# LCSL/nys-koop-lqr

Hardware: AMD Instinct MI355X
Metric: Nyström-Koopman fits/sec (K_nm build + A,B,C solve), N=1e5 m=2000 d=384 (higher is better)
Workload: dtype f64

## Files before the change

### include/nyskoop.h

```cpp
#ifndef NYSKOOP_H
#define NYSKOOP_H

#include <stdint.h>

#ifdef __cplusplus
extern "C" {
#endif

#define NK_ABI_VERSION 2

enum {
  NK_OK = 0,
  NK_ERR_BAD_ARG = -1,
  NK_ERR_HIP = -2,
  NK_ERR_NOT_SPD = -3,
  NK_ERR_OOM = -4,
  NK_ERR_NO_CONVERGENCE = -5,
  NK_ERR_NO_DEVICE = -6
};

enum { NK_KERNEL_RBF = 0, NK_KERNEL_MATERN52 = 1, NK_KERNEL_LINEAR = 2 };

typedef struct nk_kernel_desc {
  int32_t type;
// ... 40 lines not shown
int nk_set_kmat_mode(nk_ctx* ctx, int mode);
int nk_set_strict_spd(nk_ctx* ctx, int strict);
int nk_set_refine(nk_ctx* ctx, double pivot_ratio, int32_t steps);
#define NK_DTYPE_F64 0
#define NK_DTYPE_F32 1
int nk_set_compute_dtype(nk_ctx* ctx, int dtype);
int nk_wait_stream(nk_ctx* ctx, void* producer_stream);
int nk_group_create(int device, int size, nk_ctx** members);
typedef struct nk_cv_unit {
  const nk_kernel_desc* kernel;
  double gamma;
  double jitter;
  int32_t m;
  int32_t reserved;
  int64_t test_begin, test_end;
  const int64_t* landmark_rows;
} nk_cv_unit;
int nk_cv_grid(nk_ctx* const* members, int32_t n_members, const double* X, int64_t ldx, const double* Y, int64_t ldy,
               int64_t n, int32_t d, int32_t p, const nk_cv_unit* units, int32_t n_units, double* scores, int32_t* status);
int nk_group_enter(nk_ctx* member);
int nk_group_leave(nk_ctx* member);
int nk_group_stats(nk_ctx* member, uint64_t* out4);
int nk_runtime_counters(uint64_t* out, int32_t n);
int nk_shutdown(void);

void* nk_host_alloc(uint64_t bytes);
void nk_host_free(void* ptr);

int nk_kernel_matrix(nk_ctx* ctx, const nk_kernel_desc* kd,
                     const double* A, int64_t lda, int64_t nA,
                     const double* B, int64_t ldb, int64_t nB,
                     double* out, int64_t ldo);

int nk_nystrom_fit(nk_ctx* ctx, const nk_kernel_desc* kd,
                   const double* X, int64_t ldx, const double* Y, int64_t ldy,
                   int64_t n, int32_t d, int32_t p,
                   const int64_t* row_ranges, int32_t n_ranges,
                   const double* Zin, int64_t ldzi, const double* Zout, int64_t ldzo, int32_t m,
                   double gamma, double jitter,
                   nk_model** model, nk_fit_stats* stats);

int nk_gram_doubles(int32_t m, int32_t d, int32_t p, int64_t* count);
int nk_nystrom_gram(nk_ctx* ctx, const nk_kernel_desc* kd,
                    const double* X, int64_t ldx, const double* Y, int64_t ldy,
                    int64_t n, int32_t d, int32_t p,
                    const int64_t* row_ranges, int32_t n_ranges,
// ... 56 lines not shown
```

### nys_koop_lqr_amd/_lib.py

```python
import atexit
import ctypes as C
import os
import sys
import threading

import numpy as np

_HERE = os.path.dirname(os.path.abspath(__file__))

NK_KERNEL_RBF, NK_KERNEL_MATERN52, NK_KERNEL_LINEAR = 0, 1, 2
NK_OK = 0
_ERR_NAMES = {-1: "NK_ERR_BAD_ARG", -2: "NK_ERR_HIP", -3: "NK_ERR_NOT_SPD", -4: "NK_ERR_OOM",
              -5: "NK_ERR_NO_CONVERGENCE", -6: "NK_ERR_NO_DEVICE"}


class NyskoopError(RuntimeError):
    def __init__(self, code, msg):
        super().__init__(f"{_ERR_NAMES.get(code, code)}: {msg}")
        self.code = code


class KernelDesc(C.Structure):
    _fields_ = [("type", C.c_int32), ("d", C.c_int32), ("n_lengthscale", C.c_int32), ("reserved", C.c_int32),
                ("lengthscale", C.POINTER(C.c_double)), ("sigma0", C.c_double)]
# ... 22 lines not shown
_I64 = C.c_int64
_I32 = C.c_int32
_D = C.c_double

SIGNATURES = {
    "nk_version": (C.c_int, []),
    "nk_last_error": (C.c_char_p, []),
    "nk_device_count": (C.c_int, []),
    "nk_create": (C.c_int, [C.c_int, C.POINTER(_P)]),
    "nk_destroy": (C.c_int, [_P]),
    "nk_synchronize": (C.c_int, [_P]),
    "nk_stream": (_P, [_P]),
    "nk_set_kmat_mode": (C.c_int, [_P, C.c_int]),
    "nk_set_strict_spd": (C.c_int, [_P, C.c_int]),
    "nk_set_refine": (C.c_int, [_P, C.c_double, C.c_int32]),
    "nk_wait_stream": (C.c_int, [_P, _P]),
    "nk_shutdown": (C.c_int, []),
    "nk_group_create": (C.c_int, [C.c_int, C.c_int, C.POINTER(_P)]),
    "nk_group_enter": (C.c_int, [_P]),
    "nk_group_leave": (C.c_int, [_P]),
    "nk_set_compute_dtype": (C.c_int, [_P, C.c_int]),
    "nk_group_stats": (C.c_int, [_P, C.POINTER(C.c_uint64)]),
    "nk_runtime_counters": (C.c_int, [C.POINTER(C.c_uint64), C.c_int32]),
    "nk_cv_grid": (C.c_int, [C.POINTER(_P), _I32, _P, _I64, _P, _I64, _I64, _I32, _I32, C.POINTER(CvUnit), _I32,
                             C.POINTER(_D), C.POINTER(_I32)]),
    "nk_host_alloc": (_P, [C.c_uint64]),
    "nk_host_free": (None, [_P]),
    "nk_kernel_matrix": (C.c_int, [_P, C.POINTER(KernelDesc), _P, _I64, _I64, _P, _I64, _I64, _P, _I64]),
    "nk_nystrom_fit": (C.c_int, [_P, C.POINTER(KernelDesc), _P, _I64, _P, _I64, _I64, _I32, _I32,
                                 C.POINTER(_I64), _I32, _P, _I64, _P, _I64, _I32, _D, _D,
                                 C.POINTER(_P), C.POINTER(FitStats)]),
    "nk_gram_doubles": (C.c_int, [_I32, _I32, _I32, C.POINTER(_I64)]),
    "nk_nystrom_gram": (C.c_int, [_P, C.POINTER(KernelDesc), _P, _I64, _P, _I64, _I64, _I32, _I32,
                                  C.POINTER(_I64), _I32, _P, _I64, _P, _I64, _I32, _P, C.POINTER(FitStats)]),
    "nk_nystrom_solve": (C.c_int, [_P, C.POINTER(KernelDesc), _P, _I64, _P, _I64, _I32, _I32, _I32, _P, _I64, _D, _D,
                                   C.POINTER(_P), C.POINTER(FitStats)]),
    "nk_model_create": (C.c_int, [_P, C.POINTER(KernelDesc), _P, _I64, _I32, _I32, _I32, _D, _P, _P, _P, _P,
                                  C.POINTER(_P)]),
    "nk_model_destroy": (C.c_int, [_P]),
    "nk_model_get": (C.c_int, [_P, _P, C.c_char, _P, _I64]),
    "nk_model_dims": (C.c_int, [_P, C.POINTER(_I32), C.POINTER(_I32), C.POINTER(_I32)]),
    "nk_model_get_ops": (C.c_int, [_P, _P, _P, _I64, _P, _I64, _P, _I64]),
    "nk_model_get_ops_async": (C.c_int, [_P, _P, _P, _I64, _P, _I64, _P, _I64]),
    "nk_model_wait": (C.c_int, [_P]),
    "nk_lift": (C.c_int, [_P, _P, _P, _I64, _I64, _P, _I64]),
    "nk_predict": (C.c_int, [_P, _P, _P, _I64, _I64, _P, _I64]),
# ... 370 lines not shown
```

### nys_koop_lqr_amd/csrc/nk_api.hip

```cpp
#include "nk_common.h"

#include <cmath>
#include <cstdarg>
#include <cstdio>
#include <cstring>
#include <chrono>
#include <cstdlib>
#include <algorithm>
#include <condition_variable>
#include <mutex>
#include <set>
#include <thread>

namespace nk {

static thread_local std::string g_err;

void set_error(const char* fmt, ...) {
  char buf[1024];
  va_list ap;
  va_start(ap, fmt);
  vsnprintf(buf, sizeof(buf), fmt, ap);
  va_end(ap);
  g_err = buf;
// ... 520 lines not shown
    set_error("nk_group_create: could not create the shared stream / argument table");
    return NK_ERR_HIP;
  }
  for (int i = 0; i < size; ++i) group_attach(g, i, out[i]);
  return NK_OK;
}

int nk_group_enter(nk_ctx* ctx) {
  NK_REQUIRE(ctx != nullptr, "nk_group_enter: null context");
  return group_enter(ctx);
}

int nk_group_leave(nk_ctx* ctx) {
  NK_REQUIRE(ctx != nullptr, "nk_group_leave: null context");
  tl_ctx = ctx;
  const int rc = group_leave(ctx);
  tl_ctx = nullptr;
  return rc;
}

int nk_runtime_counters(uint64_t* out, int32_t n) {
  NK_REQUIRE(out != nullptr && n >= 0, "nk_runtime_counters: bad argument");
  for (int i = 0; i < n && i < CNT_N; ++i) out[i] = nk::read_counter(i);
  return NK_OK;
}

int nk_group_stats(nk_ctx* ctx, uint64_t* out4) {
  NK_REQUIRE(ctx != nullptr && out4 != nullptr, "nk_group_stats: null argument");
  group_stats(ctx, out4);
  return NK_OK;
}

int nk_cv_grid(nk_ctx* const* members, int32_t n_members, const double* X, int64_t ldx, const double* Y, int64_t ldy,
               int64_t n, int32_t d, int32_t p, const nk_cv_unit* units, int32_t n_units, double* scores, int32_t* status) {
  NK_REQUIRE(members && n_members >= 1 && X && Y && units && scores, "nk_cv_grid: null argument");
  NK_REQUIRE(n > 0 && d > 0 && p >= 0 && n_units >= 0 && ldx >= d + p && ldy >= d, "nk_cv_grid: bad sizes");
  for (int k = 0; k < n_members; ++k) NK_REQUIRE(members[k] != nullptr, "nk_cv_grid: null member context");
  for (int u = 0; u < n_units; ++u) {
    const nk_cv_unit& cu = units[u];
    NK_REQUIRE(cu.kernel && cu.landmark_rows && cu.m > 0, "nk_cv_grid: unit %d: null kernel / landmarks", u);
    NK_REQUIRE(0 <= cu.test_begin && cu.test_begin < cu.test_end && cu.test_end <= n, "nk_cv_grid: unit %d: bad test fold", u);
    for (int j = 0; j < cu.m; ++j)
      NK_REQUIRE(cu.landmark_rows[j] >= 0 && cu.landmark_rows[j] < n, "nk_cv_grid: unit %d: landmark row out of range", u);
  }
  if (n_units == 0) return NK_OK;
  nk_ctx* lead = members[0];
// ... 1562 lines not shown
```

### nys_koop_lqr_amd/csrc/nk_chol_flow.hip

```cpp
#include "nk_common.h"
#include "nk_panel_body.h"
#include "nk_potrf_body.h"

namespace nk {

namespace {

constexpr int FLOW_THREADS = 256;
constexpr int FLOW_HDR = 16;
constexpr int FLOW_POLL_LIMIT = 1 << 22;

struct FlowSys {
  double* P;
  int64_t ldp;
  int m, extra;
  double* Linv;
  double* pivlog;
  int* info;
  unsigned long long* piv;
  int* flags;
  int nblk;
  int nex;
};
struct FlowArgs {
  FlowSys s[2];
  int nsys;
  int total;
  int fix;
  int* hdr;
};

__device__ __forceinline__ int ld_flag(const int* f) { return __hip_atomic_load(f, __ATOMIC_RELAXED, __HIP_MEMORY_SCOPE_AGENT); }

__device__ __forceinline__ int col_items(const FlowSys& s, int c) {
  if (c < 0 || c >= s.nblk) return 0;
  return max(0, s.nblk - c - 2) + s.nex;
}

__device__ void item_of(const FlowArgs& a, int t, int& q, int& i, int& k) {
  for (int g = 0;; ++g) {
    for (int p = 0; p < a.nsys; ++p)
      if (g < a.s[p].nblk) {
        if (t == 0) { q = p; i = k = g; return; }
        --t;
      }
    for (int p = 0; p < a.nsys; ++p) {
      const int n = col_items(a.s[p], g - 1);
      if (t < n) {
        q = p; k = g - 1;
        const int nsq = max(0, a.s[p].nblk - k - 2);
        i = t < nsq ? k + 2 + t : a.s[p].nblk + (t - nsq);
// ... 123 lines not shown
    __hip_atomic_store(s.flags + i * s.nblk + k, 1, __ATOMIC_RELAXED, __HIP_MEMORY_SCOPE_AGENT);
  }
}

__device__ __forceinline__ void local_sync() {
  asm volatile("s_waitcnt vmcnt(0)" ::: "memory");
  __syncthreads();
}

__device__ __forceinline__ void panel_tile(const FlowArgs& a, const FlowSys& s, int r0, int r1, int k, int wave, int lane) {
  PanelSys ps;
  ps.P = s.P + (int64_t)r0 * s.ldp + CHOL_NB * k;
  ps.ldp = s.ldp;
  ps.Linv = s.Linv + (size_t)k * CHOL_WS;
  ps.rows = r1 - r0;
  ps.nb = min(CHOL_NB, s.m - CHOL_NB * k);
  ps.fix = a.fix;
  ps.nblocks = 1;
  chol_panel_rows(ps, 16 * wave, lane);
  __builtin_amdgcn_s_setprio(0);
}

__device__ __noinline__ void flow_potrf(double* A, int64_t lda, int nb, double* Linv, int* info, unsigned long long* piv,
                                       double* plog, int blk, int lane) {
  PotrfBatch pb;
  pb.A[0] = A; pb.lda[0] = lda; pb.nb[0] = nb; pb.Linv[0] = Linv; pb.info[0] = info; pb.piv[0] = piv; pb.plog[0] = plog;
  pb.A[1] = nullptr; pb.lda[1] = 0; pb.nb[1] = 0; pb.Linv[1] = nullptr; pb.info[1] = nullptr; pb.piv[1] = nullptr;
  pb.plog[1] = nullptr;
  potrf_diag_kernel_body<true>(pb, blk, 0, lane);
  __builtin_amdgcn_s_setprio(0);
}

__global__ void __launch_bounds__(FLOW_THREADS) chol_flow_kernel(FlowArgs a) {
  __shared__ int sh[4];
  const int lane = threadIdx.x & 63;
  const int wave = __builtin_amdgcn_readfirstlane(threadIdx.x >> 6);
  const int wm = wave >> 1, wn = wave & 1;
  const int l15 = lane & 15, l4 = lane >> 4;
  for (;;) {
    if (threadIdx.x == 0) sh[1] = atomicAdd(a.hdr, 1);
    __syncthreads();
    const int t = sh[1];
    __syncthreads();
    if (t >= a.total) return;
    int q = 0, i = 0, k = 0;
    item_of(a, t, q, i, k);
    const FlowSys s = q ? a.s[1] : a.s[0];
    int r0, r1;
    tile_rows(s, i, r0, r1);
    const int c0 = CHOL_NB * k, c1 = min(c0 + CHOL_NB, s.m);
    if (i == k) {
      if (k > 0) {
        const int p0 = c0 - CHOL_NB;
        Quarter Cp, Cd;
        load_quarter(s, r0, r1, p0, c0, wm, wn, l15, l4, Cp);
        load_quarter(s, r0, r1, c0, c1, wm, wn, l15, l4, Cd);
        bool ok = true;
        for (int j = 0; j < k - 1 && ok;) {
          const int J = wait_tiles(a, s, k, k - 1, j, k - 1, sh);
          if (J < 0) { ok = false; break; }
          for (; j < J; ++j) {
            update_quarter(s, r0, r1, p0, c0, j, wm, wn, l15, l4, Cp);
            update_quarter(s, r0, r1, c0, c1, j, wm, wn, l15, l4, Cd);
          }
        }
        if (!ok) continue;
        store_quarter(s, r0, r1, p0, c0, wm, wn, l15, l4, Cp);
        store_quarter(s, r0, r1, c0, c1, wm, wn, l15, l4, Cd);
        local_sync();
        if (wait_tiles(a, s, k - 1, -1, k - 1, k, sh) < 0) continue;
        panel_tile(a, s, r0, r1, k - 1, wave, lane);
        publish(s, k, k - 1);
        __syncthreads();
        load_quarter(s, r0, r1, c0, c1, wm, wn, l15, l4, Cd);
        update_quarter(s, r0, r1, c0, c1, k - 1, wm, wn, l15, l4, Cd);
        store_quarter(s, r0, r1, c0, c1, wm, wn, l15, l4, Cd);
        local_sync();
      }
      if (wave == 0)
        flow_potrf(s.P + (int64_t)c0 * s.ldp + c0, s.ldp, c1 - c0, s.Linv + (size_t)k * CHOL_WS, s.info, s.piv,
                   s.pivlog ? s.pivlog + c0 : nullptr, k, lane);
      publish(s, k, k);
      __syncthreads();
    } else {
      if (k > 0) {
        Quarter C;
        load_quarter(s, r0, r1, c0, c1, wm, wn, l15, l4, C);
        bool ok = true;
        for (int j = 0; j < k && ok;) {
          const int J = wait_tiles(a, s, i, k, j, k, sh);
          if (J < 0) { ok = false; break; }
          for (; j < J; ++j) update_quarter(s, r0, r1, c0, c1, j, wm, wn, l15, l4, C);
        }
        if (!ok) continue;
        store_quarter(s, r0, r1, c0, c1, wm, wn, l15, l4, C);
        local_sync();
      }
      if (wait_tiles(a, s, k, -1, k, k + 1, sh) < 0) continue;
      panel_tile(a, s, r0, r1, k, wave, lane);
      publish(s, i, k);
      __syncthreads();
    }
  }
}

}

bool chol_flow_enabled() {
  const char* e = getenv("NYSKOOP_CHOL_FLOW");
  return !(e && e[0] == '0');
}

int cholesky_flow_pair(nk_ctx* ctx, const CholSys* sys, int nsys) {
  constexpr int NB = CHOL_NB;
  NK_REQUIRE(nsys >= 1 && nsys <= 2, "cholesky_flow_pair: 1..2 systems");
  FlowArgs a;
  memset(&a, 0, sizeof(a));
  a.nsys = nsys;
  a.fix = chol_fix_enabled();
  size_t words = FLOW_HDR;
  for (int q = 0; q < nsys; ++q) {
    const CholSys& y = sys[q];
    FlowSys& s = a.s[q];
    s.P = y.P; s.ldp = y.ldp; s.m = y.m; s.extra = y.extra; s.Linv = y.Linv; s.pivlog = y.pivlog;
    s.info = ctx->d_info + info_base(ctx) + q;
    s.piv = ctx->d_piv + 2 * (info_base(ctx) + q);
    s.nblk = (y.m + NB - 1) / NB;
    s.nex = (y.extra + NB - 1) / NB;
    words += (size_t)(s.nblk + s.nex) * s.nblk;
    for (int c = 0; c < s.nblk; ++c) a.total += 1 + std::max(0, s.nblk - c - 2) + s.nex;
  }
  const int slot = info_base(ctx) / 2;
  if (ctx->flow_words[slot] < words) {
    if (ctx->d_flow[slot]) NK_HIP(hipFree(ctx->d_flow[slot]));
    ctx->d_flow[slot] = nullptr;
    ctx->flow_words[slot] = 0;
    NK_HIP(hipMalloc(reinterpret_cast<void**>(&ctx->d_flow[slot]), words * sizeof(int)));
    ctx->flow_words[slot] = words;
  }
  a.hdr = ctx->d_flow[slot];
  int* f = a.hdr + FLOW_HDR;
  for (int q = 0; q < nsys; ++q) {
    a.s[q].flags = f;
    f += (size_t)(a.s[q].nblk + a.s[q].nex) * a.s[q].nblk;
  }
  NK_HIP(hipMemsetAsync(a.hdr, 0, words * sizeof(int), ctx->stream));
  const int grid = std::max(1, std::min(a.total, ctx->num_cu / 2));
  hipLaunchKernelGGL(chol_flow_kernel, dim3((unsigned)grid), dim3(FLOW_THREADS), 0, ctx->stream, a);
  NK_HIP(hipGetLastError());
  count_event(CNT_CHOL_FLOW);
  return NK_OK;
}

}
```

### nys_koop_lqr_amd/csrc/nk_common.h

```cpp
#pragma once
#include <hip/hip_runtime.h>
#include <stdint.h>
#include <stddef.h>
#include <string>
#include <vector>

#include "nyskoop.h"
#include "nk_lockstep.h"

namespace nk {

void set_error(const char* fmt, ...);

#define NK_HIP(call)                                                                         \
  do {                                                                                       \
    hipError_t e_ = (call);                                                                  \
    if (e_ != hipSuccess) {                                                                  \
      nk::set_error("%s failed: %s (%s:%d)", #call, hipGetErrorString(e_), __FILE__, __LINE__); \
      return e_ == hipErrorOutOfMemory ? NK_ERR_OOM : NK_ERR_HIP;                            \
    }                                                                                        \
  } while (0)

#define NK_TRY(call)            \
  do {                          \
// ... 39 lines not shown
  hipStream_t stream_la[2] = {nullptr, nullptr};
  hipEvent_t ev_la[2][4] = {};
  int compute_f32 = 0;
  hipEvent_t ev_fork = nullptr, ev_join = nullptr, ev_chain = nullptr;
  int* d_info = nullptr;
  unsigned long long* d_piv = nullptr;
  unsigned long long* h_piv = nullptr;
  double* d_scalars = nullptr;
  double* h_scalars = nullptr;
  int* h_info = nullptr;
  double* d_zeros = nullptr;
  hipEvent_t ev[16];
  int num_cu = 256;
  int kmat_mode = 0;
  double refine_pivot = 0.0;
  int refine_steps = 2;
  int strict_spd = 0;
  hipEvent_t ev_ext = nullptr;
  hipEvent_t ev_up[8] = {};
  nk_group* group = nullptr;
  nk_member_state* gstate = nullptr;
  int* d_flow[2] = {nullptr, nullptr};
  size_t flow_words[2] = {0, 0};
  bool chol_flow_off = false;
  double* h_stage = nullptr;
  size_t h_stage_bytes = 0;
};

struct nk_model {
  int device = 0;
  int32_t m = 0, d = 0, p = 0;
  int32_t ktype = 0;
  double sigma0 = 0.0;
  double jitter = 0.0;
  double* buf = nullptr;
  size_t bytes = 0;
  double *A = nullptr, *B = nullptr, *C = nullptr, *W = nullptr, *S = nullptr, *Sinv = nullptr, *Z = nullptr,
         *winv = nullptr;
  bool has_ops = false;
  hipEvent_t ev_fetch = nullptr;
};

namespace nk {

struct SideScope {
  nk_ctx* c;
// ... 131 lines not shown
int sqrtm_finish(nk_ctx* ctx, SqrtPlan* plan, double* S, double* Sinv);
int sqrtm_verdict(nk_ctx* ctx, SqrtPlan* plan, int* iters, double* resid);
int cholesky_lower(nk_ctx* ctx, double* P, int64_t ldp, int m, double* Linv );
int cholesky_solve(nk_ctx* ctx, const double* L, int64_t ldl, int m, const double* Linv, double* R, int64_t ldr,
                   int nrhs);
struct CholSys {
  double* P = nullptr;
  int64_t ldp = 0;
  int m = 0;
  int extra = 0;
  bool backward = true;
  double* Linv = nullptr;
  double* pivlog = nullptr;
  double* R = nullptr;
  int64_t ldr = 0;
  int nrhs = 0;
};
int cholesky_lower_pair(nk_ctx* ctx, const CholSys* sys, int nsys);
int cholesky_lower_pair_async(nk_ctx* ctx, const CholSys* sys, int nsys);
int cholesky_check_pair(nk_ctx* ctx, const CholSys* sys, int nsys);
int cholesky_solve_pair(nk_ctx* ctx, const CholSys* sys, int nsys);
int cholesky_aug_pair_async(nk_ctx* ctx, const CholSys* sys, int nsys, hipEvent_t pause = nullptr, int pause_step = -1);
constexpr int CHOL_NB = 64;
constexpr int CHOL_WS = 2 * CHOL_NB * CHOL_NB + 8;
constexpr double CHOL_FIX_KAPPA = 8.0 * CHOL_NB;
inline int chol_fix_enabled() {
  const char* e = getenv("NYSKOOP_CHOL_FIX");
  return (e && e[0] == '0') ? 0 : ((e && e[0] == '2') ? 2 : 1);
}
bool launch_chol_trail_pair(nk_ctx* ctx, const GemmCall* calls, int ncalls, int* rc);
bool launch_chol_trail_potrf_pair(nk_ctx* ctx, const GemmCall* calls, int ncalls, const int* nb, double* const* Linv, int blk,
                                  double* const* plog, int* rc);
inline bool chol_fuse_enabled() {
  const char* e = getenv("NYSKOOP_CHOL_FUSE");
  return !(e && e[0] == '0');
}
bool chol_flow_enabled();
int cholesky_flow_pair(nk_ctx* ctx, const CholSys* sys, int nsys);
constexpr int CHOL_FLOW_GIVEUP = -0x40000000;
bool launch_chol_panel_pair(nk_ctx* ctx, const GemmCall* calls, int ncalls, int* rc);
int launch_trsm_right_lower_pair(nk_ctx* ctx, const CholSys* sys, int nsys);

struct PinvInfo {
  int rank = 0, sweeps = 0;
  bool converged = false;
  double sigma_max = 0.0, sigma_min_kept = 0.0, sigma_min = 0.0;
// ... 130 lines not shown
```

### nys_koop_lqr_amd/csrc/nk_potrf_body.h

```cpp
#pragma once
#include "nk_common.h"

namespace nk {

typedef double d4 __attribute__((ext_vector_type(4)));

__device__ __forceinline__ double readlane_f64(double v, int lane) {
  const int lo = __builtin_amdgcn_readlane(__double2loint(v), lane);
  const int hi = __builtin_amdgcn_readlane(__double2hiint(v), lane);
  return __hiloint2double(hi, lo);
}

struct PotrfBatch {
  double* A[2];
  int64_t lda[2];
  int nb[2];
  double* Linv[2];
  int* info[2];
  unsigned long long* piv[2];
  double* plog[2];
};

constexpr int PLD = CHOL_NB + 1;
constexpr int SLD = 17;
// ... 5 lines not shown
    double a = P[l15 * ldp + 4 * ks + l4];
    const double b = Q[(4 * ks + l4) * ldq + l15];
    if (NEG) a = -a;
    acc = __builtin_amdgcn_mfma_f64_16x16x4f64(a, b, acc, 0, 0, 0);
  }
  return acc;
}
__device__ __forceinline__ void store_tile(double* T, int ldt, d4 acc, int l15, int l4) {
#pragma unroll
  for (int reg = 0; reg < 4; ++reg) T[(l4 + 4 * reg) * ldt + l15] = acc[reg];
}

template <bool WAVE_SYNC>
__device__ __forceinline__ void potrf_sync() {
  if (WAVE_SYNC) {
    __builtin_amdgcn_fence(__ATOMIC_RELEASE, "workgroup");
    __builtin_amdgcn_wave_barrier();
    __builtin_amdgcn_fence(__ATOMIC_ACQUIRE, "workgroup");
  } else {
    __syncthreads();
  }
}

template <bool WAVE_SYNC = false>
__device__ __forceinline__ void potrf_diag_kernel_body(const PotrfBatch& pb, int blk, int which, int lane) {
  constexpr int NB = CHOL_NB;
  static_assert(NB == 64, "one lane per row, four 16-column panels");
  const int nb = pb.nb[which];
  if (nb <= 0) return;
  __builtin_amdgcn_s_setprio(3);
  double* __restrict__ A = pb.A[which];
  const int64_t lda = pb.lda[which];
  double* __restrict__ Linv = pb.Linv[which];
  int* __restrict__ info = pb.info[which];
  double* __restrict__ plog = pb.plog[which];
  double piv_min = 1.0e308, piv_max = 0.0;
  __shared__ double As[NB * PLD];
  __shared__ double Iv[NB * PLD];
  __shared__ double Sc[3 * 16 * SLD];
  __shared__ double dinv[NB];
  const int l15 = lane & 15, l4 = lane >> 4;
#pragma unroll 8
  for (int r = 0; r < NB; ++r) {
    double v = (r == lane) ? 1.0 : 0.0;
    if (r < nb && lane < nb) v = A[(int64_t)r * lda + lane];
    As[r * PLD + lane] = v;
  }
  potrf_sync<WAVE_SYNC>();

#pragma unroll
  for (int pbk = 0; pbk < 4; ++pbk) {
    const int c0 = 16 * pbk;
    double R[16];
#pragma unroll
    for (int jj = 0; jj < 16; ++jj) R[jj] = As[lane * PLD + c0 + jj];
#pragma unroll
    for (int k = 0; k < 16; ++k) {
      double dkk = readlane_f64(R[k], c0 + k);
      if (lane == 0 && plog != nullptr && c0 + k < nb) plog[c0 + k] = dkk;
      if (!(dkk > 0.0) || !isfinite(dkk)) {
        if (lane == 0 && c0 + k < nb) atomicCAS(info, 0, blk * NB + c0 + k + 1);
        dkk = 1.0;
      } else if (c0 + k < nb) {
        piv_min = fmin(piv_min, dkk);
        piv_max = fmax(piv_max, dkk);
      }
      double inv = __builtin_amdgcn_rsq(dkk);
      inv = inv * fma(-0.5 * dkk * inv, inv, 1.5);
      inv = inv * fma(-0.5 * dkk * inv, inv, 1.5);
      double s = dkk * inv;
      s = fma(0.5 * inv, fma(-s, s, dkk), s);
      inv = fma(inv, fma(-s, inv, 1.0), inv);
      if (lane == c0 + k) dinv[c0 + k] = inv;
      R[k] = (lane == c0 + k) ? s : R[k] * inv;
      {
        const int rk_lo = __double2loint(R[k]), rk_hi = __double2hiint(R[k]);
#pragma unroll
        for (int jj = k + 1; jj < 16; ++jj)
          asm volatile("v_readlane_b32 s96, %1, %3\n\tv_readlane_b32 s97, %2, %3\n\ts_nop 0\n\tv_fma_f64 %0, -%4, s[96:97], %0"
                       : "+v"(R[jj])
                       : "v"(rk_lo), "v"(rk_hi), "i"(c0 + jj), "v"(R[k])
                       : "s96", "s97");
      }
    }
#pragma unroll
    for (int jj = 0; jj < 16; ++jj) As[lane * PLD + c0 + jj] = R[jj];
    potrf_sync<WAVE_SYNC>();
#pragma unroll
    for (int ti = pbk + 1; ti < 4; ++ti)
#pragma unroll
      for (int tj = pbk + 1; tj <= ti; ++tj) {
        d4 c;
#pragma unroll
        for (int reg = 0; reg < 4; ++reg) c[reg] = As[(16 * ti + l4 + 4 * reg) * PLD + 16 * tj + l15];
#pragma unroll
        for (int ks = 0; ks < 4; ++ks) {
          const double a = -As[(16 * ti + l15) * PLD + c0 + 4 * ks + l4];
          const double b = As[(16 * tj + l15) * PLD + c0 + 4 * ks + l4];
          c = __builtin_amdgcn_mfma_f64_16x16x4f64(a, b, c, 0, 0, 0);
        }
#pragma unroll
        for (int reg = 0; reg < 4; ++reg) As[(16 * ti + l4 + 4 * reg) * PLD + 16 * tj + l15] = c[reg];
      }
    potrf_sync<WAVE_SYNC>();
  }
#pragma unroll 8
  for (int r = 0; r < NB; ++r)
    if (r < nb && lane < nb) A[(int64_t)r * lda + lane] = As[r * PLD + lane];

  {
    const double* Lb = As + (16 * l4) * PLD + 16 * l4;
    double x[16];
#pragma unroll
    for (int i = 0; i < 16; ++i) {
      double s0 = (i == l15) ? 1.0 : 0.0, s1 = 0.0;
#pragma unroll
      for (int j = 0; j < i; ++j) {
        const double l = Lb[i * PLD + j];
        if ((j & 1) == 0) s0 = fma(-l, x[j], s0);
        else s1 = fma(-l, x[j], s1);
      }
      x[i] = (s0 + s1) * dinv[16 * l4 + i];
    }
    double* Db = Iv + (16 * l4) * PLD + 16 * l4;
#pragma unroll
    for (int i = 0; i < 16; ++i) Db[i * PLD + l15] = x[i];
  }
  potrf_sync<WAVE_SYNC>();
  auto Lblk = [&](int i, int j) { return As + (16 * i) * PLD + 16 * j; };
  auto Xblk = [&](int i, int j) { return Iv + (16 * i) * PLD + 16 * j; };
  const d4 zero = d4{0.0, 0.0, 0.0, 0.0};
#pragma unroll
  for (int i = 1; i < 4; ++i)
    store_tile(Sc + (i - 1) * 16 * SLD, SLD, mm16<false>(Lblk(i, i - 1), PLD, Xblk(i - 1, i - 1), PLD, zero, l15, l4), l15, l4);
  potrf_sync<WAVE_SYNC>();
#pragma unroll
  for (int i = 1; i < 4; ++i)
    store_tile(Xblk(i, i - 1), PLD, mm16<true>(Xblk(i, i), PLD, Sc + (i - 1) * 16 * SLD, SLD, zero, l15, l4), l15, l4);
  potrf_sync<WAVE_SYNC>();
#pragma unroll
  for (int i = 2; i < 4; ++i) {
    d4 t = mm16<false>(Lblk(i, i - 2), PLD, Xblk(i - 2, i - 2), PLD, zero, l15, l4);
    t = mm16<false>(Lblk(i, i - 1), PLD, Xblk(i - 1, i - 2), PLD, t, l15, l4);
    store_tile(Sc + (i - 2) * 16 * SLD, SLD, t, l15, l4);
  }
  potrf_sync<WAVE_SYNC>();
#pragma unroll
  for (int i = 2; i < 4; ++i)
    store_tile(Xblk(i, i - 2), PLD, mm16<true>(Xblk(i, i), PLD, Sc + (i - 2) * 16 * SLD, SLD, zero, l15, l4), l15, l4);
  potrf_sync<WAVE_SYNC>();
  {
    d4 t = mm16<false>(Lblk(3, 0), PLD, Xblk(0, 0), PLD, zero, l15, l4);
    t = mm16<false>(Lblk(3, 1), PLD, Xblk(1, 0), PLD, t, l15, l4);
    t = mm16<false>(Lblk(3, 2), PLD, Xblk(2, 0), PLD, t, l15, l4);
    store_tile(Sc, SLD, t, l15, l4);
  }
  potrf_sync<WAVE_SYNC>();
  store_tile(Xblk(3, 0), PLD, mm16<true>(Xblk(3, 3), PLD, Sc, SLD, zero, l15, l4), l15, l4);
  potrf_sync<WAVE_SYNC>();
#pragma unroll 8
  for (int i = 0; i < NB; ++i) Linv[i * NB + lane] = (l4 <= (i >> 4)) ? Iv[i * PLD + lane] : 0.0;
  double sl = 0.0, si = 0.0;
#pragma unroll 8
  for (int i = 0; i < NB; ++i) {
    const double vl = (lane <= i) ? As[i * PLD + lane] : 0.0;
    const double vi = (l4 <= (i >> 4)) ? Iv[i * PLD + lane] : 0.0;
    Linv[NB * NB + i * NB + lane] = vl;
    sl = fma(vl, vl, sl);
    si = fma(vi, vi, si);
  }
#pragma unroll
  for (int off = 32; off > 0; off >>= 1) {
    sl += __shfl_xor(sl, off, 64);
    si += __shfl_xor(si, off, 64);
  }
  if (lane == 0) Linv[2 * NB * NB] = (sl * si > CHOL_FIX_KAPPA * CHOL_FIX_KAPPA) ? 1.0 : 0.0;
  if (lane == 0 && piv_max > 0.0) {
    atomicMin(pb.piv[which], (unsigned long long)__double_as_longlong(piv_min));
    atomicMax(pb.piv[which] + 1, (unsigned long long)__double_as_longlong(piv_max));
  }
}
}
```

Baseline: 24.49.

## Factor flow diagonal block with all four waves, keeping updated tile in LDS

By default the Cholesky flow kernel now factors each diagonal 64x64 block with all four waves instead of wave 0 alone. The panel factorisation on wave 0 runs alongside the blocked triangular inverse on wave 1, and the trailing MFMA tile updates are spread across waves. The updated diagonal quarter now stays in LDS rather than making a round-trip through global memory, and is written back only after publish. Optional wall-clock stamps and an nk_flow_stamps API are added for profiling, and the old single-wave path is kept behind NYSKOOP_FLOW_DIAG=1. The catch is extra __syncthreads inside the block and a more complex dependency order in the inverse computation.

```diff
diff --git a/include/nyskoop.h b/include/nyskoop.h
--- a/include/nyskoop.h
+++ b/include/nyskoop.h
@@ -86,6 +86,7 @@
 int nk_group_leave(nk_ctx* member);
 int nk_group_stats(nk_ctx* member, uint64_t* out4);
 int nk_runtime_counters(uint64_t* out, int32_t n);
+int nk_flow_stamps(nk_ctx* ctx, int32_t slot, uint64_t* out, int32_t n, int32_t* meta);
 int nk_shutdown(void);
 
 void* nk_host_alloc(uint64_t bytes);
diff --git a/nys_koop_lqr_amd/_lib.py b/nys_koop_lqr_amd/_lib.py
--- a/nys_koop_lqr_amd/_lib.py
+++ b/nys_koop_lqr_amd/_lib.py
@@ -68,6 +68,7 @@
     "nk_set_compute_dtype": (C.c_int, [_P, C.c_int]),
     "nk_group_stats": (C.c_int, [_P, C.POINTER(C.c_uint64)]),
     "nk_runtime_counters": (C.c_int, [C.POINTER(C.c_uint64), C.c_int32]),
+    "nk_flow_stamps": (C.c_int, [_P, _I32, C.POINTER(C.c_uint64), _I32, C.POINTER(_I32)]),
     "nk_cv_grid": (C.c_int, [C.POINTER(_P), _I32, _P, _I64, _P, _I64, _I64, _I32, _I32, C.POINTER(CvUnit), _I32,
                              C.POINTER(_D), C.POINTER(_I32)]),
     "nk_host_alloc": (_P, [C.c_uint64]),
diff --git a/nys_koop_lqr_amd/csrc/nk_api.hip b/nys_koop_lqr_amd/csrc/nk_api.hip
--- a/nys_koop_lqr_amd/csrc/nk_api.hip
+++ b/nys_koop_lqr_amd/csrc/nk_api.hip
@@ -566,6 +566,29 @@
 int nk_runtime_counters(uint64_t* out, int32_t n) {
   NK_REQUIRE(out != nullptr && n >= 0, "nk_runtime_counters: bad argument");
   for (int i = 0; i < n && i < CNT_N; ++i) out[i] = nk::read_counter(i);
+  return NK_OK;
+}
+
+int nk_flow_stamps(nk_ctx* ctx, int32_t slot, uint64_t* out, int32_t n, int32_t* meta) {
+  NK_TRY(check_ctx(ctx));
+  NK_REQUIRE(slot >= 0 && slot < 2 && out != nullptr && n >= 0 && meta != nullptr, "nk_flow_stamps: bad argument");
+  NK_HIP(hipSetDevice(ctx->device));
+  for (hipStream_t q : {ctx->stream_main, ctx->stream_side, ctx->stream_prep})
+    if (q) NK_HIP(hipStreamSynchronize(q));
+  const bool on = ctx->flow_stamp_off[slot] != 0;
+  meta[0] = on ? ctx->flow_stamp_nblk[slot][0] : 0;
+  meta[1] = on ? ctx->flow_stamp_nblk[slot][1] : 0;
+  meta[2] = FLOW_NST;
+  int khz = 0;
+  NK_HIP(hipDeviceGetAttribute(&khz, hipDeviceAttributeWallClockRate, ctx->device));
+  meta[3] = khz;
+  const size_t total = (size_t)(meta[0] + meta[1]) * FLOW_NST;
+  if (on && total > 0 && n > 0)
+  {
+    NK_HIP(hipMemcpyAsync(out, ctx->d_flow[slot] + ctx->flow_stamp_off[slot], std::min(total, (size_t)n) * sizeof(uint64_t),
+                          hipMemcpyDeviceToHost, ctx->stream_main));
+    NK_HIP(hipStreamSynchronize(ctx->stream_main));
+  }
   return NK_OK;
 }
 
diff --git a/nys_koop_lqr_amd/csrc/nk_chol_flow.hip b/nys_koop_lqr_amd/csrc/nk_chol_flow.hip
--- a/nys_koop_lqr_amd/csrc/nk_chol_flow.hip
+++ b/nys_koop_lqr_amd/csrc/nk_chol_flow.hip
@@ -21,12 +21,14 @@
   int* flags;
   int nblk;
   int nex;
+  unsigned long long* stamps;
 };
 struct FlowArgs {
   FlowSys s[2];
   int nsys;
   int total;
   int fix;
+  int diag1;
   int* hdr;
 };
 
@@ -196,13 +198,65 @@
 }
 
 __device__ __noinline__ void flow_potrf(double* A, int64_t lda, int nb, double* Linv, int* info, unsigned long long* piv,
-                                       double* plog, int blk, int lane) {
+                                       double* plog, int blk, int lane, unsigned long long* st) {
   PotrfBatch pb;
   pb.A[0] = A; pb.lda[0] = lda; pb.nb[0] = nb; pb.Linv[0] = Linv; pb.info[0] = info; pb.piv[0] = piv; pb.plog[0] = plog;
   pb.A[1] = nullptr; pb.lda[1] = 0; pb.nb[1] = 0; pb.Linv[1] = nullptr; pb.info[1] = nullptr; pb.piv[1] = nullptr;
   pb.plog[1] = nullptr;
-  potrf_diag_kernel_body<true>(pb, blk, 0, lane);
+  potrf_diag_kernel_body<true>(pb, blk, 0, lane, st);
   __builtin_amdgcn_s_setprio(0);
+}
+
+__device__ __forceinline__ void flow_diag_load(const double* A, int64_t lda, int nb, int wave, int lane) {
+  double* As = potrf_lds().As;
+#pragma unroll
+  for (int rr = 0; rr < 16; ++rr) {
+    const int r = 16 * wave + rr;
+    double v = (r == lane) ? 1.0 : 0.0;
+    if (r < nb && lane < nb) v = A[(int64_t)r * lda + lane];
+    As[r * PLD + lane] = v;
+  }
+}
+__device__ __noinline__ void flow_diag4(const double* A, int64_t lda, int nb, double* Linv, int* info, unsigned long long* piv,
+                                        double* plog, int blk, int wave, int lane, unsigned long long* st) {
+  if (A != nullptr) flow_diag_load(A, lda, nb, wave, lane);
+  __syncthreads();
+  potrf_stamp(st, 4);
+  potrf_diag_flow_body(nb, Linv, info, piv, plog, blk, wave, lane, st);
+  __builtin_amdgcn_s_setprio(0);
+}
+
+template <bool PAD>
+__device__ __forceinline__ void quarter_to_lds(const Quarter& C, int nb, int wm, int wn, int l15, int l4) {
+  double* As = potrf_lds().As;
+#pragma unroll
+  for (int a = 0; a < 2; ++a)
+#pragma unroll
+    for (int b = 0; b < 2; ++b)
+#pragma unroll
+      for (int reg = 0; reg < 4; ++reg) {
+        const int row = 32 * wm + 16 * a + l4 + 4 * reg, col = 32 * wn + 16 * b + l15;
+        double v = C[a][b][reg];
+        if (PAD && !(row < nb && col < nb)) v = (row == col) ? 1.0 : 0.0;
+        As[row * PLD + col] = v;
+      }
+}
+__device__ __forceinline__ void quarter_from_lds(Quarter& C, int wm, int wn, int l15, int l4) {
+  const double* As = potrf_lds().As;
+#pragma unroll
+  for (int a = 0; a < 2; ++a)
+#pragma unroll
+    for (int b = 0; b < 2; ++b)
+#pragma unroll
+      for (int reg = 0; reg < 4; ++reg) C[a][b][reg] = As[(32 * wm + 16 * a + l4 + 4 * reg) * PLD + 32 * wn + 16 * b + l15];
+}
+__device__ __forceinline__ void flow_diag_writeback(double* A, int64_t lda, int nb, int wave, int lane) {
+  const double* As = potrf_lds().As;
+#pragma unroll
+  for (int rr = 0; rr < 16; ++rr) {
+    const int r = 16 * wave + rr;
+    if (r < nb && lane < nb) A[(int64_t)r * lda + lane] = As[r * PLD + lane];
+  }
 }
 
 __global__ void __launch_bounds__(FLOW_THREADS) chol_flow_kernel(FlowArgs a) {
@@ -224,6 +278,10 @@
     tile_rows(s, i, r0, r1);
     const int c0 = CHOL_NB * k, c1 = min(c0 + CHOL_NB, s.m);
     if (i == k) {
+      unsigned long long* st = s.stamps ? s.stamps + (size_t)k * FLOW_NST : nullptr;
+      potrf_stamp(st, 0);
+      const int nb = c1 - c0;
+      double* Akk = s.P + (int64_t)c0 * s.ldp + c0;
       if (k > 0) {
         const int p0 = c0 - CHOL_NB;
         Quarter Cp, Cd;
@@ -239,23 +297,42 @@
           }
         }
         if (!ok) continue;
+        potrf_stamp(st, 1);
         store_quarter(s, r0, r1, p0, c0, wm, wn, l15, l4, Cp);
-        store_quarter(s, r0, r1, c0, c1, wm, wn, l15, l4, Cd);
+        if (a.diag1) store_quarter(s, r0, r1, c0, c1, wm, wn, l15, l4, Cd);
+        else quarter_to_lds<false>(Cd, nb, wm, wn, l15, l4);
         local_sync();
         if (wait_tiles(a, s, k - 1, -1, k - 1, k, sh) < 0) continue;
+        potrf_stamp(st, 2);
         panel_tile(a, s, r0, r1, k - 1, wave, lane);
         publish(s, k, k - 1);
         __syncthreads();
-        load_quarter(s, r0, r1, c0, c1, wm, wn, l15, l4, Cd);
-        update_quarter(s, r0, r1, c0, c1, k - 1, wm, wn, l15, l4, Cd);
-        store_quarter(s, r0, r1, c0, c1, wm, wn, l15, l4, Cd);
-        local_sync();
-      }
-      if (wave == 0)
-        flow_potrf(s.P + (int64_t)c0 * s.ldp + c0, s.ldp, c1 - c0, s.Linv + (size_t)k * CHOL_WS, s.info, s.piv,
-                   s.pivlog ? s.pivlog + c0 : nullptr, k, lane);
+        potrf_stamp(st, 3);
+        if (a.diag1) {
+          load_quarter(s, r0, r1, c0, c1, wm, wn, l15, l4, Cd);
+          update_quarter(s, r0, r1, c0, c1, k - 1, wm, wn, l15, l4, Cd);
+          store_quarter(s, r0, r1, c0, c1, wm, wn, l15, l4, Cd);
+          local_sync();
+        } else {
+          quarter_from_lds(Cd, wm, wn, l15, l4);
+          update_quarter(s, r0, r1, c0, c1, k - 1, wm, wn, l15, l4, Cd);
+          quarter_to_lds<true>(Cd, nb, wm, wn, l15, l4);
+        }
+      }
+      double* plog = s.pivlog ? s.pivlog + c0 : nullptr;
+      double* Lk = s.Linv + (size_t)k * CHOL_WS;
+      if (a.diag1) {
+        if (wave == 0) flow_potrf(Akk, s.ldp, nb, Lk, s.info, s.piv, plog, k, lane, st);
+      } else {
+        flow_diag4(k == 0 ? Akk : nullptr, s.ldp, nb, Lk, s.info, s.piv, plog, k, wave, lane, st);
+      }
       publish(s, k, k);
       __syncthreads();
+      potrf_stamp(st, 10);
+      if (!a.diag1) {
+        flow_diag_writeback(Akk, s.ldp, nb, wave, lane);
+        potrf_stamp(st, 11);
+      }
     } else {
       if (k > 0) {
         Quarter C;
@@ -280,6 +357,11 @@
 
 }
 
+static bool env_is_1(const char* name) {
+  const char* e = getenv(name);
+  return e && e[0] == '1';
+}
+
 bool chol_flow_enabled() {
   const char* e = getenv("NYSKOOP_CHOL_FLOW");
   return !(e && e[0] == '0');
@@ -292,6 +374,8 @@
   memset(&a, 0, sizeof(a));
   a.nsys = nsys;
   a.fix = chol_fix_enabled();
+  a.diag1 = env_is_1("NYSKOOP_FLOW_DIAG");
+  const bool stamps = env_is_1("NYSKOOP_FLOW_STAMPS");
   size_t words = FLOW_HDR;
   for (int q = 0; q < nsys; ++q) {
     const CholSys& y = sys[q];
@@ -302,6 +386,7 @@
     s.nblk = (y.m + NB - 1) / NB;
     s.nex = (y.extra + NB - 1) / NB;
     words += (size_t)(s.nblk + s.nex) * s.nblk;
+    if (stamps) words += 2 * (size_t)s.nblk * FLOW_NST + 1;
     for (int c = 0; c < s.nblk; ++c) a.total += 1 + std::max(0, s.nblk - c - 2) + s.nex;
   }
   const int slot = info_base(ctx) / 2;
@@ -318,6 +403,18 @@
     a.s[q].flags = f;
     f += (size_t)(a.s[q].nblk + a.s[q].nex) * a.s[q].nblk;
   }
+  ctx->flow_stamp_off[slot] = 0;
+  if (stamps) {
+    ctx->flow_stamp_off[slot] = (f - a.hdr + 1) & ~(size_t)1;
+    unsigned long long* st = reinterpret_cast<unsigned long long*>(a.hdr + ctx->flow_stamp_off[slot]);
+    for (int q = 0; q < 2; ++q) {
+      ctx->flow_stamp_nblk[slot][q] = q < nsys ? a.s[q].nblk : 0;
+      if (q < nsys) {
+        a.s[q].stamps = st;
+        st += (size_t)a.s[q].nblk * FLOW_NST;
+      }
+    }
+  }
   NK_HIP(hipMemsetAsync(a.hdr, 0, words * sizeof(int), ctx->stream));
   const int grid = std::max(1, std::min(a.total, ctx->num_cu / 2));
   hipLaunchKernelGGL(chol_flow_kernel, dim3((unsigned)grid), dim3(FLOW_THREADS), 0, ctx->stream, a);
diff --git a/nys_koop_lqr_amd/csrc/nk_common.h b/nys_koop_lqr_amd/csrc/nk_common.h
--- a/nys_koop_lqr_amd/csrc/nk_common.h
+++ b/nys_koop_lqr_amd/csrc/nk_common.h
@@ -85,6 +85,8 @@
   nk_member_state* gstate = nullptr;
   int* d_flow[2] = {nullptr, nullptr};
   size_t flow_words[2] = {0, 0};
+  size_t flow_stamp_off[2] = {0, 0};
+  int flow_stamp_nblk[2][2] = {{0, 0}, {0, 0}};
   bool chol_flow_off = false;
   double* h_stage = nullptr;
   size_t h_stage_bytes = 0;
@@ -262,6 +264,7 @@
 int cholesky_solve_pair(nk_ctx* ctx, const CholSys* sys, int nsys);
 int cholesky_aug_pair_async(nk_ctx* ctx, const CholSys* sys, int nsys, hipEvent_t pause = nullptr, int pause_step = -1);
 constexpr int CHOL_NB = 64;
+constexpr int FLOW_NST = 16;
 constexpr int CHOL_WS = 2 * CHOL_NB * CHOL_NB + 8;
 constexpr double CHOL_FIX_KAPPA = 8.0 * CHOL_NB;
 inline int chol_fix_enabled() {
diff --git a/nys_koop_lqr_amd/csrc/nk_potrf_body.h b/nys_koop_lqr_amd/csrc/nk_potrf_body.h
--- a/nys_koop_lqr_amd/csrc/nk_potrf_body.h
+++ b/nys_koop_lqr_amd/csrc/nk_potrf_body.h
@@ -51,8 +51,100 @@
   }
 }
 
+struct PotrfLds {
+  double As[CHOL_NB * PLD];
+  double Iv[CHOL_NB * PLD];
+  double Sc[3 * 16 * SLD];
+  double dinv[CHOL_NB];
+};
+__device__ __forceinline__ PotrfLds& potrf_lds() {
+  __shared__ PotrfLds s;
+  return s;
+}
+
+__device__ __forceinline__ void potrf_stamp(unsigned long long* st, int slot) {
+  if (st != nullptr && threadIdx.x == 0) st[slot] = (unsigned long long)wall_clock64();
+}
+
+__device__ __forceinline__ void potrf_panel(double* As, double* dinv, int pbk, int lane, int nb, int blk, int* info, double* plog,
+                                            double& piv_min, double& piv_max) {
+  constexpr int NB = CHOL_NB;
+  const int c0 = 16 * pbk;
+  double R[16];
+#pragma unroll
+  for (int jj = 0; jj < 16; ++jj) R[jj] = As[lane * PLD + c0 + jj];
+#pragma unroll
+  for (int k = 0; k < 16; ++k) {
+    double dkk = readlane_f64(R[k], c0 + k);
+    if (lane == 0 && plog != nullptr && c0 + k < nb) plog[c0 + k] = dkk;
+    if (!(dkk > 0.0) || !isfinite(dkk)) {
+      if (lane == 0 && c0 + k < nb) atomicCAS(info, 0, blk * NB + c0 + k + 1);
+      dkk = 1.0;
+    } else if (c0 + k < nb) {
+      piv_min = fmin(piv_min, dkk);
+      piv_max = fmax(piv_max, dkk);
+    }
+    double inv = __builtin_amdgcn_rsq(dkk);
+    inv = inv * fma(-0.5 * dkk * inv, inv, 1.5);
+    inv = inv * fma(-0.5 * dkk * inv, inv, 1.5);
+    double s = dkk * inv;
+    s = fma(0.5 * inv, fma(-s, s, dkk), s);
+    inv = fma(inv, fma(-s, inv, 1.0), inv);
+    if (lane == c0 + k) dinv[c0 + k] = inv;
+    R[k] = (lane == c0 + k) ? s : R[k] * inv;
+    {
+      const int rk_lo = __double2loint(R[k]), rk_hi = __double2hiint(R[k]);
+#pragma unroll
+      for (int jj = k + 1; jj < 16; ++jj)
+        asm volatile("v_readlane_b32 s96, %1, %3\n\tv_readlane_b32 s97, %2, %3\n\ts_nop 0\n\tv_fma_f64 %0, -%4, s[96:97], %0"
+                     : "+v"(R[jj])
+                     : "v"(rk_lo), "v"(rk_hi), "i"(c0 + jj), "v"(R[k])
+                     : "s96", "s97");
+    }
+  }
+#pragma unroll
+  for (int jj = 0; jj < 16; ++jj) As[lane * PLD + c0 + jj] = R[jj];
+}
+
+__device__ __forceinline__ void potrf_tile_update(double* As, int pbk, int ti, int tj, int l15, int l4) {
+  const int c0 = 16 * pbk;
+  d4 c;
+#pragma unroll
+  for (int reg = 0; reg < 4; ++reg) c[reg] = As[(16 * ti + l4 + 4 * reg) * PLD + 16 * tj + l15];
+#pragma unroll
+  for (int ks = 0; ks < 4; ++ks) {
+    const double a = -As[(16 * ti + l15) * PLD + c0 + 4 * ks + l4];
+    const double b = As[(16 * tj + l15) * PLD + c0 + 4 * ks + l4];
+    c = __builtin_amdgcn_mfma_f64_16x16x4f64(a, b, c, 0, 0, 0);
+  }
+#pragma unroll
+  for (int reg = 0; reg < 4; ++reg) As[(16 * ti + l4 + 4 * reg) * PLD + 16 * tj + l15] = c[reg];
+}
+
+__device__ __forceinline__ void potrf_inv_diag(const double* As, double* Iv, const double* dinv, int b, int l15, bool store) {
+  const double* Lb = As + (16 * b) * PLD + 16 * b;
+  double x[16];
+#pragma unroll
+  for (int i = 0; i < 16; ++i) {
+    double s0 = (i == l15) ? 1.0 : 0.0, s1 = 0.0;
+#pragma unroll
+    for (int j = 0; j < i; ++j) {
+      const double l = Lb[i * PLD + j];
+      if ((j & 1) == 0) s0 = fma(-l, x[j], s0);
+      else s1 = fma(-l, x[j], s1);
+    }
+    x[i] = (s0 + s1) * dinv[16 * b + i];
+  }
+  if (store) {
+    double* Db = Iv + (16 * b) * PLD + 16 * b;
+#pragma unroll
+    for (int i = 0; i < 16; ++i) Db[i * PLD + l15] = x[i];
+  }
+}
+
 template <bool WAVE_SYNC = false>
-__device__ __forceinline__ void potrf_diag_kernel_body(const PotrfBatch& pb, int blk, int which, int lane) {
+__device__ __forceinline__ void potrf_diag_kernel_body(const PotrfBatch& pb, int blk, int which, int lane,
+                                                       unsigned long long* st = nullptr) {
   constexpr int NB = CHOL_NB;
   static_assert(NB == 64, "one lane per row, four 16-column panels");
   const int nb = pb.nb[which];
@@ -64,10 +156,11 @@
   int* __restrict__ info = pb.info[which];
   double* __restrict__ plog = pb.plog[which];
   double piv_min = 1.0e308, piv_max = 0.0;
-  __shared__ double As[NB * PLD];
-  __shared__ double Iv[NB * PLD];
-  __shared__ double Sc[3 * 16 * SLD];
-  __shared__ double dinv[NB];
+  PotrfLds& lds = potrf_lds();
+  double* As = lds.As;
+  double* Iv = lds.Iv;
+  double* Sc = lds.Sc;
+  double* dinv = lds.dinv;
   const int l15 = lane & 15, l4 = lane >> 4;
 #pragma unroll 8
   for (int r = 0; r < NB; ++r) {
@@ -76,85 +169,24 @@
     As[r * PLD + lane] = v;
   }
   potrf_sync<WAVE_SYNC>();
+  potrf_stamp(st, 4);
 
 #pragma unroll
   for (int pbk = 0; pbk < 4; ++pbk) {
-    const int c0 = 16 * pbk;
-    double R[16];
-#pragma unroll
-    for (int jj = 0; jj < 16; ++jj) R[jj] = As[lane * PLD + c0 + jj];
-#pragma unroll
-    for (int k = 0; k < 16; ++k) {
-      double dkk = readlane_f64(R[k], c0 + k);
-      if (lane == 0 && plog != nullptr && c0 + k < nb) plog[c0 + k] = dkk;
-      if (!(dkk > 0.0) || !isfinite(dkk)) {
-        if (lane == 0 && c0 + k < nb) atomicCAS(info, 0, blk * NB + c0 + k + 1);
-        dkk = 1.0;
-      } else if (c0 + k < nb) {
-        piv_min = fmin(piv_min, dkk);
-        piv_max = fmax(piv_max, dkk);
-      }
-      double inv = __builtin_amdgcn_rsq(dkk);
-      inv = inv * fma(-0.5 * dkk * inv, inv, 1.5);
-      inv = inv * fma(-0.5 * dkk * inv, inv, 1.5);
-      double s = dkk * inv;
-      s = fma(0.5 * inv, fma(-s, s, dkk), s);
-      inv = fma(inv, fma(-s, inv, 1.0), inv);
-      if (lane == c0 + k) dinv[c0 + k] = inv;
-      R[k] = (lane == c0 + k) ? s : R[k] * inv;
-      {
-        const int rk_lo = __double2loint(R[k]), rk_hi = __double2hiint(R[k]);
-#pragma unroll
-        for (int jj = k + 1; jj < 16; ++jj)
-          asm volatile("v_readlane_b32 s96, %1, %3\n\tv_readlane_b32 s97, %2, %3\n\ts_nop 0\n\tv_fma_f64 %0, -%4, s[96:97], %0"
-                       : "+v"(R[jj])
-                       : "v"(rk_lo), "v"(rk_hi), "i"(c0 + jj), "v"(R[k])
-                       : "s96", "s97");
-      }
-    }
-#pragma unroll
-    for (int jj = 0; jj < 16; ++jj) As[lane * PLD + c0 + jj] = R[jj];
+    potrf_panel(As, dinv, pbk, lane, nb, blk, info, plog, piv_min, piv_max);
     potrf_sync<WAVE_SYNC>();
 #pragma unroll
     for (int ti = pbk + 1; ti < 4; ++ti)
 #pragma unroll
-      for (int tj = pbk + 1; tj <= ti; ++tj) {
-        d4 c;
-#pragma unroll
-        for (int reg = 0; reg < 4; ++reg) c[reg] = As[(16 * ti + l4 + 4 * reg) * PLD + 16 * tj + l15];
-#pragma unroll
-        for (int ks = 0; ks < 4; ++ks) {
-          const double a = -As[(16 * ti + l15) * PLD + c0 + 4 * ks + l4];
-          const double b = As[(16 * tj + l15) * PLD + c0 + 4 * ks + l4];
-          c = __builtin_amdgcn_mfma_f64_16x16x4f64(a, b, c, 0, 0, 0);
-        }
-#pragma unroll
-        for (int reg = 0; reg < 4; ++reg) As[(16 * ti + l4 + 4 * reg) * PLD + 16 * tj + l15] = c[reg];
-      }
+      for (int tj = pbk + 1; tj <= ti; ++tj) potrf_tile_update(As, pbk, ti, tj, l15, l4);
     potrf_sync<WAVE_SYNC>();
+    potrf_stamp(st, 5 + pbk);
   }
 #pragma unroll 8
   for (int r = 0; r < NB; ++r)
     if (r < nb && lane < nb) A[(int64_t)r * lda + lane] = As[r * PLD + lane];
 
-  {
-    const double* Lb = As + (16 * l4) * PLD + 16 * l4;
-    double x[16];
-#pragma unroll
-    for (int i = 0; i < 16; ++i) {
-      double s0 = (i == l15) ? 1.0 : 0.0, s1 = 0.0;
-#pragma unroll
-      for (int j = 0; j < i; ++j) {
-        const double l = Lb[i * PLD + j];
-        if ((j & 1) == 0) s0 = fma(-l, x[j], s0);
-        else s1 = fma(-l, x[j], s1);
-      }
-      x[i] = (s0 + s1) * dinv[16 * l4 + i];
-    }
-    double* Db = Iv + (16 * l4) * PLD + 16 * l4;
-#pragma unroll
-    for (int i = 0; i < 16; ++i) Db[i * PLD + l15] = x[i];
-  }
+  potrf_inv_diag(As, Iv, dinv, l4, l15, true);
   potrf_sync<WAVE_SYNC>();
   auto Lblk = [&](int i, int j) { return As + (16 * i) * PLD + 16 * j; };
   auto Xblk = [&](int i, int j) { return Iv + (16 * i) * PLD + 16 * j; };
@@ -187,6 +219,7 @@
   potrf_sync<WAVE_SYNC>();
   store_tile(Xblk(3, 0), PLD, mm16<true>(Xblk(3, 3), PLD, Sc, SLD, zero, l15, l4), l15, l4);
   potrf_sync<WAVE_SYNC>();
+  potrf_stamp(st, 9);
 #pragma unroll 8
   for (int i = 0; i < NB; ++i) Linv[i * NB + lane] = (l4 <= (i >> 4)) ? Iv[i * PLD + lane] : 0.0;
   double sl = 0.0, si = 0.0;
@@ -209,4 +242,98 @@
     atomicMax(pb.piv[which] + 1, (unsigned long long)__double_as_longlong(piv_max));
   }
 }
-}
+
+__device__ __forceinline__ void potrf_diag_flow_body(int nb, double* Linv, int* info, unsigned long long* piv, double* plog,
+                                                     int blk, int wave, int lane, unsigned long long* st) {
+  constexpr int NB = CHOL_NB;
+  __builtin_amdgcn_s_setprio(3);
+  PotrfLds& lds = potrf_lds();
+  double* As = lds.As;
+  double* Iv = lds.Iv;
+  double* dinv = lds.dinv;
+  const int l15 = lane & 15, l4 = lane >> 4;
+  double piv_min = 1.0e308, piv_max = 0.0;
+  auto Lblk = [&](int i, int j) { return As + (16 * i) * PLD + 16 * j; };
+  auto Xblk = [&](int i, int j) { return Iv + (16 * i) * PLD + 16 * j; };
+  auto Sblk = [&](int i, int j) { return Iv + (16 * j) * PLD + 16 * i; };
+  const d4 zero = d4{0.0, 0.0, 0.0, 0.0};
+
+#pragma unroll
+  for (int pbk = 0; pbk < 4; ++pbk) {
+    if (wave == 0) {
+      potrf_panel(As, dinv, pbk, lane, nb, blk, info, plog, piv_min, piv_max);
+    } else if (wave == 1 && pbk > 0) {
+      const int p = pbk - 1;
+      potrf_inv_diag(As, Iv, dinv, p, l15, l4 == 0);
+      potrf_sync<true>();
+      if (p == 0) {
+        store_tile(Sblk(1, 0), PLD, mm16<false>(Lblk(1, 0), PLD, Xblk(0, 0), PLD, zero, l15, l4), l15, l4);
+      } else if (p == 1) {
+        store_tile(Xblk(1, 0), PLD, mm16<true>(Xblk(1, 1), PLD, Sblk(1, 0), PLD, zero, l15, l4), l15, l4);
+        store_tile(Sblk(2, 1), PLD, mm16<false>(Lblk(2, 1), PLD, Xblk(1, 1), PLD, zero, l15, l4), l15, l4);
+        potrf_sync<true>();
+        d4 t = mm16<false>(Lblk(2, 0), PLD, Xblk(0, 0), PLD, zero, l15, l4);
+        t = mm16<false>(Lblk(2, 1), PLD, Xblk(1, 0), PLD, t, l15, l4);
+        store_tile(Sblk(2, 0), PLD, t, l15, l4);
+      } else {
+        store_tile(Xblk(2, 1), PLD, mm16<true>(Xblk(2, 2), PLD, Sblk(2, 1), PLD, zero, l15, l4), l15, l4);
+        store_tile(Xblk(2, 0), PLD, mm16<true>(Xblk(2, 2), PLD, Sblk(2, 0), PLD, zero, l15, l4), l15, l4);
+        store_tile(Sblk(3, 2), PLD, mm16<false>(Lblk(3, 2), PLD, Xblk(2, 2), PLD, zero, l15, l4), l15, l4);
+        potrf_sync<true>();
+        d4 t = mm16<false>(Lblk(3, 1), PLD, Xblk(1, 1), PLD, zero, l15, l4);
+        t = mm16<false>(Lblk(3, 2), PLD, Xblk(2, 1), PLD, t, l15, l4);
+        store_tile(Sblk(3, 1), PLD, t, l15, l4);
+        t = mm16<false>(Lblk(3, 0), PLD, Xblk(0, 0), PLD, zero, l15, l4);
+        t = mm16<false>(Lblk(3, 1), PLD, Xblk(1, 0), PLD, t, l15, l4);
+        t = mm16<false>(Lblk(3, 2), PLD, Xblk(2, 0), PLD, t, l15, l4);
+        store_tile(Sblk(3, 0), PLD, t, l15, l4);
+      }
+    }
+    __syncthreads();
+    if (pbk < 3) {
+      int t = 0;
+#pragma unroll
+      for (int ti = pbk + 1; ti < 4; ++ti)
+#pragma unroll
+        for (int tj = pbk + 1; tj <= ti; ++tj, ++t)
+          if ((t & 3) == wave) potrf_tile_update(As, pbk, ti, tj, l15, l4);
+      __syncthreads();
+    }
+    potrf_stamp(st, 5 + pbk);
+  }
+
+  if (wave == 0) {
+    potrf_inv_diag(As, Iv, dinv, 3, l15, l4 == 0);
+    potrf_sync<true>();
+#pragma unroll
+    for (int j = 0; j < 3; ++j)
+      store_tile(Xblk(3, j), PLD, mm16<true>(Xblk(3, 3), PLD, Sblk(3, j), PLD, zero, l15, l4), l15, l4);
+  } else {
+    for (int i = wave - 1; i < NB; i += 3) Linv[NB * NB + i * NB + lane] = (lane <= i) ? As[i * PLD + lane] : 0.0;
+    for (int i = wave - 1; i < 48; i += 3) Linv[i * NB + lane] = (l4 <= (i >> 4)) ? Iv[i * PLD + lane] : 0.0;
+  }
+  __syncthreads();
+  potrf_stamp(st, 9);
+  for (int i = 48 + wave; i < NB; i += 4) Linv[i * NB + lane] = Iv[i * PLD + lane];
+  if (wave == 1) {
+    double sl = 0.0, si = 0.0;
+#pragma unroll 8
+    for (int i = 0; i < NB; ++i) {
+      const double vl = (lane <= i) ? As[i * PLD + lane] : 0.0;
+      const double vi = (l4 <= (i >> 4)) ? Iv[i * PLD + lane] : 0.0;
+      sl = fma(vl, vl, sl);
+      si = fma(vi, vi, si);
+    }
+#pragma unroll
+    for (int off = 32; off > 0; off >>= 1) {
+      sl += __shfl_xor(sl, off, 64);
+      si += __shfl_xor(si, off, 64);
+    }
+    if (lane == 0) Linv[2 * NB * NB] = (sl * si > CHOL_FIX_KAPPA * CHOL_FIX_KAPPA) ? 1.0 : 0.0;
+  }
+  if (wave == 0 && lane == 0 && piv_max > 0.0) {
+    atomicMin(piv, (unsigned long long)__double_as_longlong(piv_min));
+    atomicMax(piv + 1, (unsigned long long)__double_as_longlong(piv_max));
+  }
+}
+}
```

New measurement: 24.71 (median of 6 runs). About the same (+0.9%).
